# mhozza/covest

Measured on AMD Instinct MI355X. Metric: grid-point log-likelihood evals/s, repeat model, 10k-bin hist, higher is better.
Workload: dtype f64

## Files before the change

covest_amd/csrc/abi_grid.cpp:

```cpp
#include "host.h"

using namespace covest;

namespace covest {

int grid_stage_begin(covest_grid *g, size_t bytes, StageSlot &slot)
{
    if (!g->async_uploads) {
        SharedStage &ss = shared_stage();
        slot.shared_hold = std::unique_lock<std::mutex>(ss.mu);
        HIP_TRY(ss.buf.reserve(bytes));
        slot.ptr = ss.buf.as<char>();
        return COVEST_OK;
    }
    const size_t at = (g->stage_off + 63) / 64 * 64;
    if (at + bytes > g->stage.cap) {
        if (g->stage.ptr)
            g->stage_retired.push_back(std::move(g->stage));
        HIP_TRY(g->stage.reserve(std::max<size_t>(2 * (at + bytes), 1 << 18)));
        slot.ptr = g->stage.as<char>();
        g->stage_off = bytes;
        return COVEST_OK;
    }
    slot.ptr = g->stage.as<char>() + at;
// ... 15 lines not shown

}

namespace {

int check_grid_args(const covest_model *m, int32_t n_axes, const double *const *axes, const int64_t *axis_len, int64_t flat_begin,
                    int64_t *flat_end, const char *who, int64_t *total_out, int64_t *n_values_out)
{
    if (!axes || !axis_len)
        return fail(COVEST_E_INVALID, std::string(who) + ": null argument");
    if (n_axes != m->n_par)
        return fail(COVEST_E_INVALID, std::string(who) + ": n_axes must equal the model's param_count");
    int64_t total = 1, n_values = 0;
    for (int d = 0; d < n_axes; ++d) {
        if (axis_len[d] < 1 || !axes[d])
            return fail(COVEST_E_INVALID, std::string(who) + ": every axis needs at least one value");
        if (total > (int64_t)1 << 40)
            return fail(COVEST_E_INVALID, std::string(who) + ": grid too large");
        total *= axis_len[d];
        n_values += axis_len[d];
    }
    if (*flat_end < 0)
        *flat_end = total;
    if (flat_begin < 0 || flat_begin > *flat_end || *flat_end > total)
        return fail(COVEST_E_INVALID, std::string(who) + ": bad flat index range");
    *total_out = total;
    *n_values_out = n_values;
    return COVEST_OK;
}

struct GridArena {
    size_t ctl, axes, table;
    size_t staged_bytes;
    size_t ll, idx, word, partial_val, partial_idx, result, bytes;
    GridArena(int64_t n_values, int64_t nq, int64_t n)
    {
        const size_t n_pts = (size_t)(n > 0 ? n : 1);
        ctl = 0;
        axes = 8;
        table = axes + (size_t)n_values * sizeof(double);
        staged_bytes = (table + (size_t)nq * sizeof(int32_t) + 7) / 8 * 8;
        ll = staged_bytes;
        idx = ll + n_pts * sizeof(double);
        word = idx + n_pts * sizeof(int64_t);
        partial_val = word + n_pts * sizeof(unsigned long long);
        partial_idx = partial_val + kArgminBlocks * sizeof(double);
        result = partial_idx + kArgminBlocks * sizeof(int64_t);
        bytes = result + sizeof(ArgminResult);
    }
};

int stage_inputs(covest_grid *g, const GridArena &a, int32_t n_axes, const double *const *axes, const int64_t *axis_len,
                 const std::vector<int32_t> &table, int64_t n, char **inputs)
{
    const void *arena_before = g->arena.ptr;
    const bool counter_clean = g->counter_clean;
    HIP_TRY(g->arena.reserve(a.bytes));
    char *base = g->arena.as<char>();
    StageSlot slot;
    const int src = grid_stage_begin(g, a.staged_bytes, slot);
    if (src != COVEST_OK)
        return src;
    char *stage = slot.ptr;
    std::memset(stage, 0, a.staged_bytes);
    double *sa = reinterpret_cast<double *>(stage + a.axes);
    for (int d = 0; d < n_axes; ++d) {
        std::copy(axes[d], axes[d] + axis_len[d], sa);
        sa += axis_len[d];
    }
    if (!table.empty())
        std::memcpy(stage + a.table, table.data(), table.size() * sizeof(int32_t));
    if (g->async_uploads && n <= kArgminSmall) {
        *inputs = stage;
        if (!(counter_clean && g->arena.ptr == arena_before && g->sub_ctl.ptr == base + a.ctl)) {
            HIP_TRY(hipMemsetAsync(base + a.ctl, 0, 8, nullptr));
            g->upload_pending = true;
        }
        return COVEST_OK;
    }
    *inputs = base;
    return grid_stage_commit(g, slot, base, a.staged_bytes);
}

void bind_views(covest_grid *g, const GridArena &a, char *inputs, int32_t n_axes, const int64_t *axis_len, int64_t flat_begin)
{
    char *base = g->arena.as<char>();
    g->axes.ptr = inputs + a.axes;
    g->sub_ctl.ptr = base + a.ctl;
    g->t_table.ptr = inputs + a.table;
    g->ll.ptr = base + a.ll;
    g->sub_index.ptr = base + a.idx;
    g->sub_word.ptr = base + a.word;
    g->partial_val.ptr = base + a.partial_val;
    g->partial_idx.ptr = base + a.partial_idx;
    g->result.ptr = base + a.result;
    PointSource &src = g->src;
    src = PointSource{};
    src.is_grid = 1;
    src.flat_begin = flat_begin;
    int64_t off = 0;
    for (int d = 0; d < kMaxParams; ++d) {
        g->len[d] = src.len[d] = d < n_axes ? axis_len[d] : 1;
        src.axis[d] = d < n_axes ? g->axes.as<double>() + off : nullptr;
        if (d < n_axes)
            off += axis_len[d];
    }
    if (g->model->n_par == 5)
        src.t_table = g->t_table.as<int32_t>();
}

struct TMinus1Sums {
    double block, q;
};

TMinus1Sums sum_t_minus_1(const std::vector<int32_t> &table, int64_t nq, int64_t flat_begin, int64_t flat_end)
{
    std::vector<double> prefix((size_t)nq + 1, 0.0);
    for (int64_t i = 0; i < nq; ++i)
        prefix[(size_t)i + 1] = prefix[(size_t)i] + (double)(table[(size_t)i] > 1 ? table[(size_t)i] - 1 : 0);
    auto upto = [&](int64_t flat) {
        return (double)(flat / nq) * prefix[(size_t)nq] + prefix[(size_t)(flat % nq)];
    };
    return {upto(flat_end) - upto(flat_begin), prefix[(size_t)nq]};
}

// ... 64 lines not shown
        pinned_block_give(g->result_host);
        g->result_host = nullptr;
    }
    g->arena.release();
    g->plan_buf.release();
    g->axis_buf.release();
    g->axis_host.release();
    for (covest_grid::Part &part : g->long_parts)
        part.buf.release();
    g->long_parts.clear();
    g->long_q_orig.release();
    g->long_partial.release();
    for (hipEvent_t e : g->ev_begin)
        (void)hipEventDestroy(e);
    for (hipEvent_t e : g->ev_end)
        (void)hipEventDestroy(e);
    g->ev_begin.clear();
    g->ev_end.clear();
}

extern "C" {

int covest_grid_create(covest_model *m, int32_t n_axes, const double *const *axes,
                       const int64_t *axis_len, int64_t flat_begin, int64_t flat_end,
                       covest_grid **out)
{
    if (!m || !out)
        return fail(COVEST_E_INVALID, "covest_grid_create: null argument");
    *out = nullptr;
    covest_grid *g = new (std::nothrow) covest_grid();
    if (!g)
        return fail(COVEST_E_NOMEM, "covest_grid_create: out of host memory");
    g->model = m;
    std::lock_guard<std::mutex> guard(m->lock);
    DeviceGuard dev_guard(m->device);
    int rc = dev_guard.status();
    if (rc == COVEST_OK)
        rc = grid_configure(g, n_axes, axes, axis_len, flat_begin, flat_end, "covest_grid_create");
    if (rc != COVEST_OK) {
        grid_release(g);
        delete g;
        return rc;
    }
    *out = g;
    return COVEST_OK;
}

int covest_grid_reset(covest_grid *g, int32_t n_axes, const double *const *axes, const int64_t *axis_len,
                      int64_t flat_begin, int64_t flat_end)
{
    if (!g)
        return fail(COVEST_E_INVALID, "covest_grid_reset: null grid");
    covest_model *m = g->model;
    std::lock_guard<std::mutex> guard(m->lock);
    DeviceGuard dev_guard(m->device);
    if (dev_guard.status() != COVEST_OK)
        return dev_guard.status();
    if (g->last_stream || g->evaluated)
        HIP_TRY(hipStreamSynchronize(g->last_stream));
    if (g->upload_pending && !g->evaluated)
        HIP_TRY(hipStreamSynchronize(nullptr));
    g->upload_pending = false;
    g->stage_retired.clear();
    g->async_uploads = true;
    return grid_configure(g, n_axes, axes, axis_len, flat_begin, flat_end, "covest_grid_reset");
}
// ... 75 lines not shown
    for (unsigned long long w : words) {
        const long long unit = sub_units16(w) ? 16 : 1;
        const long long len = ((long long)sub_last(w) - (long long)sub_first(w) + 1) * unit;
        sum += (double)len;
        mx = std::max(mx, len);
        mn = std::min(mn, len);
        first_sum += (long long)sub_first(w) * unit;
    }
    std::fprintf(stderr, "covest_grid_eval: rows named per point: min %lld mean %.1f max %lld; mean first row %.1f\n", mn,
                 sum / queued, mx, (double)first_sum / queued);
    if (!g->src.t_table)
        return COVEST_OK;
    const int64_t n_q = g->src.len[2] * g->src.len[3] * g->src.len[4];
    std::vector<int32_t> tt((size_t)n_q);
    std::vector<int64_t> idx(queued);
    HIP_TRY(hipMemcpy(tt.data(), g->src.t_table, (size_t)n_q * sizeof(int32_t), hipMemcpyDeviceToHost));
    HIP_TRY(hipMemcpy(idx.data(), g->sub_index.ptr, (size_t)queued * sizeof(int64_t), hipMemcpyDeviceToHost));
    long long tmin = 1 << 30, tmax = 0;
    double tsum = 0;
    long long hist[6] = {0, 0, 0, 0, 0, 0};
    for (int64_t i : idx) {
        const long long T = tt[(size_t)((g->src.flat_begin + i) % n_q)];
        tmin = std::min(tmin, T);
        tmax = std::max(tmax, T);
        tsum += (double)T;
        hist[T <= 16 ? 0 : T <= 32 ? 1 : T <= 64 ? 2 : T <= 128 ? 3 : T <= 256 ? 4 : 5]++;
    }
    std::fprintf(stderr, "covest_grid_eval: threshold_o of the queued points: min %lld mean %.1f max %lld; <=16 %lld <=32 %lld <=64 %lld <=128 %lld <=256 %lld more %lld\n",
                 tmin, tsum / queued, tmax, hist[0], hist[1], hist[2], hist[3], hist[4], hist[5]);
    return COVEST_OK;
}
#endif

static int grid_eval(covest_grid *g, int32_t kernel, void *stream, bool scan, double scan_start)
{
    if (!g)
        return fail(COVEST_E_INVALID, "covest_grid_eval: null grid");
    if (!g->configured)
        return fail(COVEST_E_INVALID, "covest_grid_eval: the last covest_grid_reset of this handle failed; reset it again");
    covest_model *m = g->model;
    const int kern = resolve_kernel(m, kernel, g);
    if (kern < 0)
        return kern;
    std::lock_guard<std::mutex> guard(m->lock);
    DeviceGuard dev_guard(m->device);
    int rc = dev_guard.status();
    if (rc != COVEST_OK)
        return rc;
    LaunchRecordScope record(g->record);
    hipStream_t st = static_cast<hipStream_t>(stream);
    const int64_t n = g->flat_end - g->flat_begin;
    if (g->upload_pending && st != nullptr && g->upload_ev)
        HIP_TRY(hipStreamWaitEvent(st, g->upload_ev, 0));
    hipEvent_t bracket_end = nullptr;
    rc = bracket_begin(g, st, &bracket_end);
    if (rc != COVEST_OK)
        return rc;
    HIP_TRY(launch_ll(m, kern, g->src, n, g->ll.as<double>(), sub_list_of(m, g->has_plan ? g->t_max : 2, g->sub_index.ptr, g->sub_word.ptr, g->sub_ctl.ptr), st,
                      &g->last_kernel, g));
    g->last_kernel_id = kern;
    if (bracket_end)
        HIP_TRY(hipEventRecord(bracket_end, st));
#ifdef COVEST_DIAG
    rc = report_queue(g, st, n);
    if (rc != COVEST_OK)
        return rc;
#endif
    if (!g->result_host) {
        static_assert(sizeof(ArgminResult) <= 64 && 64 + sizeof(ScanRecords) <= kPinnedBlockBytes, "pinned block");
        g->result_host = static_cast<ArgminResult *>(pinned_block_take());
        if (!g->result_host)
            return fail(COVEST_E_NOMEM, "covest_grid_eval: no page-locked memory for the result");
    }
    g->scan_valid = scan && n >= 1 && n <= kArgminSmall;
    if (g->scan_valid)
        HIP_TRY(launch_argmin_scan(g->ll.as<double>(), n, g->flat_begin, scan_start, g->result.as<ArgminResult>(), g->result_host,
                                   g->scan_host(), g->sub_ctl.as<unsigned>(), st));
    else
        HIP_TRY(launch_argmin(g->ll.as<double>(), n, g->flat_begin, g->partial_val.as<double>(),
                              g->partial_idx.as<int64_t>(), g->result.as<ArgminResult>(), g->result_host, g->sub_ctl.as<unsigned>(), st));
    g->last_stream = st;
    g->evaluated = true;
    return COVEST_OK;
}

int covest_grid_eval(covest_grid *g, int32_t kernel, void *stream) { return grid_eval(g, kernel, stream, false, 0.0); }

int covest_grid_eval_scan(covest_grid *g, int32_t kernel, void *stream, double start_min)
{
    return grid_eval(g, kernel, stream, true, start_min);
}

int covest_grid_scan(covest_grid *g, int32_t cap, int64_t *index, double *negll, int32_t *n_records, int32_t *truncated)
{
    if (!g || !n_records || !truncated || cap < 0 || (cap > 0 && (!index || !negll)))
        return fail(COVEST_E_INVALID, "covest_grid_scan: bad argument");
    if (!g->evaluated)
        return fail(COVEST_E_INVALID, "covest_grid_scan: covest_grid_eval_scan has not run");
    DeviceGuard dev_guard(g->model->device);
    int rc = dev_guard.status();
    if (rc != COVEST_OK)
        return rc;
    HIP_TRY(hipStreamSynchronize(g->last_stream));
    *n_records = 0;
    *truncated = 1;
    if (!g->scan_valid)
        return COVEST_OK;
    const ScanRecords *sr = g->scan_host();
    const int32_t have = sr->n;
    *truncated = (sr->truncated || have > cap) ? 1 : 0;
// ... 145 lines not shown
```

covest_amd/csrc/argmin.hip:

```cpp
#include <hip/hip_runtime.h>

#include <algorithm>

#include "cand.h"
#include "direct_point.h"
#include "fastmath.h"
#include "kernels.h"
#include "wave.h"

namespace covest {

namespace {

__device__ __forceinline__ Cand block_best(Cand c)
{
    __shared__ double sv[16];
    __shared__ int64_t si[16];
    c = wave_best(c);
    const int lane = threadIdx.x & (kWave - 1), w = threadIdx.x / kWave;
    if (lane == 0) {
        sv[w] = c.v;
        si[w] = c.i;
    }
    __syncthreads();
// ... 130 lines not shown
                                if (u >= n)
                                    break;
                                if (idx[u] >= cur_end) {
                                    if (cur_end > 0)
                                        pj += wave_bcast(b_o, cur_end - S) * inner;
                                    inner = 0.0;
                                    while (idx[u] >= cur_end)
                                        cur_end += S;
                                }
                                inner += t[u];
                            }
                        }
                        if (cur_end > 0)
                            pj += wave_bcast(b_o, cur_end - S) * inner;
                    }
                }
            }
            if (NW > 1) {
                pj_part[wave][lane] = pj;
                __syncthreads();
                pj = ((pj_part[0][lane] + pj_part[1][lane]) + pj_part[2][lane]) + pj_part[3][lane];
            }
            const bool fix = counted && pj < list.p_clamp;
            const double contrib = fix ? h * ((pj <= 0.0 ? -INFINITY : log(pj)) - list.log_p_clamp) : 0.0;
            uint64_t todo = __ballot(fix);
            while (todo) {
                const int kk = __builtin_ctzll(todo);
                todo &= todo - 1;
                value += wave_bcast(contrib, kk);
            }
            if (NW > 1)
                __syncthreads();
        }
        if (lane == 0 && wave == 0)
            ll[pt] = value;
    }
}

template <int SC>
__global__ __launch_bounds__(256) void ll_fix_basic_packed_kernel(const DevModel m, const int32_t n_tiles, const int32_t n_items,
                                                                  const double *__restrict__ tile_dbl,
                                                                  const int32_t *__restrict__ tile_int, const PointSource src,
                                                                  double *__restrict__ ll, const SubList list)
{
    const unsigned count = __builtin_amdgcn_readfirstlane(*list.count);
    if (count == 0)
        return;
    __shared__ __attribute__((aligned(16))) double log_tab[kLogTableDoubles];
    load_log_table(log_tab);
    const TileView tv = tile_view_from(n_tiles, n_items, tile_dbl, tile_int);
    const int lane = threadIdx.x & (kWave - 1);
    constexpr int S = SC;
    constexpr int G = kWave / S;
    const int g = lane / S, s = lane - g * S;
    const bool in_group = g < G;
    const int first_lane = (in_group ? g : 0) * S;
    const double comb_s = m.comb[s];
    const int64_t n_rows_table = (int64_t)tv.n_tiles * kTileBins;
    const unsigned wave_global = blockIdx.x * (blockDim.x / kWave) + threadIdx.x / kWave;
    const unsigned n_waves = gridDim.x * (blockDim.x / kWave);
    bool have = false;
    int64_t pt = 0, row_first = 0, row_last = -1;
    double par[kMaxParams] = {0, 0, 0, 0, 0};
    int T = 0;
    double value = 0.0, h_n = 0.0, key_n = 0.0, nlg_n = 0.0;
    auto fetch_row = [&](int64_t r0, double &h, double &key, double &nlg) {
        const int64_t row = row_first + r0 + s;
        const int bin = (have && row <= row_last && row < n_rows_table) ? tv.row_bin[row] : -1;
// ... 37 lines not shown
            nd = -log_trunc_norm(x, lx, log_tab);
        }
        if (!live)
            a_s = 0.0;
        const int64_t my_rows = have ? row_last - row_first + 1 : 0;
        int64_t most = my_rows;
#pragma unroll
        for (int off = 32; off >= 1; off >>= 1)
            most = max(most, __shfl_xor(most, off, kWave));
        for (int64_t r0 = 0; r0 < most; r0 += S) {
            const double h = h_n, key = key_n, nlg = nlg_n;
            if (r0 + S < most)
                fetch_row(r0 + S, h_n, key_n, nlg_n);
            const bool counted = h != 0.0;
            double pj = 0.0;
#pragma unroll
            for (int t = 0; t < S; ++t) {
                const double a_t = __shfl(a_s, first_lane + t, kWave);
                const double lx_t = __shfl(lx, first_lane + t, kWave);
                const double nd_t = __shfl(nd, first_lane + t, kWave);
                const double term = a_t * exp(fma(key, lx_t, nd_t + nlg));
                pj += (a_t != 0.0) ? term : 0.0;
            }
            const bool fix = counted && pj < list.p_clamp;
            const double contrib = fix ? h * ((pj <= 0.0 ? -INFINITY : log(pj)) - list.log_p_clamp) : 0.0;
#pragma unroll
            for (int t = 0; t < S; ++t) {
                const double c_t = __shfl(contrib, first_lane + t, kWave);
                const bool f_t = __shfl((int)fix, first_lane + t, kWave) != 0;
                if (f_t)
                    value += c_t;
            }
        }
        if (have && s == 0)
            ll[pt] = value;
    }
}

__device__ __forceinline__ void publish(Cand c, int64_t flat_begin, ArgminResult *__restrict__ result,
                                        ArgminResult *__restrict__ host_mirror)
{
    ArgminResult r;
    r.min_negll = c.v;
    r.index = (c.i == INT64_MAX) ? -1 : c.i;
    r.pair[0] = c.v;
    r.pair[1] = (c.i == INT64_MAX) ? -1.0 : (double)(flat_begin + c.i);
    *result = r;
    if (host_mirror)
        *host_mirror = r;
}

__global__ __launch_bounds__(256) void argmin_stage2(const double *__restrict__ pv,
                                                     const int64_t *__restrict__ pi, int n_part, int64_t flat_begin,
                                                     ArgminResult *__restrict__ result, ArgminResult *__restrict__ host_mirror,
                                                     unsigned *__restrict__ queue_count)
{
    if (threadIdx.x == 0 && queue_count)
        *queue_count = 0;
    Cand c;
    c.v = INFINITY;
    c.i = INT64_MAX;
    for (int i = threadIdx.x; i < n_part; i += blockDim.x) {
        Cand o;
        o.v = pv[i];
        o.i = pi[i];
        c = better(c, o);
    }
    c = block_best(c);
// ... 10 lines not shown
        double v[4];
#pragma unroll
        for (int u = 0; u < 4; ++u) {
            const int64_t i = base + (int64_t)u * kSmallThreads;
            v[u] = i < n ? -ll[i] : INFINITY;
        }
#pragma unroll
        for (int u = 0; u < 4; ++u) {
            const int64_t i = base + (int64_t)u * kSmallThreads;
            if (i < n)
                take(i, v[u]);
        }
    }
}

__global__ __launch_bounds__(kSmallThreads) void argmin_small(const double *__restrict__ ll, int64_t n, int64_t flat_begin,
                                                             ArgminResult *__restrict__ result, ArgminResult *__restrict__ host_mirror,
                                                             unsigned *__restrict__ queue_count)
{
    if (threadIdx.x == 0 && queue_count)
        *queue_count = 0;
    Cand c;
    c.v = INFINITY;
    c.i = INT64_MAX;
    small_grid_values(ll, n, [&](int64_t i, double v) {
        if (v < c.v) {
            c.v = v;
            c.i = i;
        }
    });
    c = block_best(c);
    if (threadIdx.x == 0)
        publish(c, flat_begin, result, host_mirror);
}

__global__ __launch_bounds__(kSmallThreads) void argmin_scan_small(const double *__restrict__ ll, int64_t n, int64_t flat_begin,
                                                                  double start, ArgminResult *__restrict__ result,
                                                                  ArgminResult *__restrict__ host_mirror,
                                                                  ScanRecords *__restrict__ scan, unsigned *__restrict__ queue_count)
{
    constexpr int NW = kSmallThreads / kWave;
    extern __shared__ double vals[];
    __shared__ double wave_min[NW];
    __shared__ int wave_cnt[NW];
    const int tid = threadIdx.x, lane = tid & (kWave - 1), w = tid / kWave;
    if (tid == 0 && queue_count)
        *queue_count = 0;
    Cand c;
    c.v = INFINITY;
    c.i = INT64_MAX;
    small_grid_values(ll, n, [&](int64_t i, double v) {
        vals[i] = v;
        if (v < c.v) {
            c.v = v;
            c.i = i;
        }
    });
    c = block_best(c);
    if (tid == 0)
        publish(c, flat_begin, result, host_mirror);
    const int chunk = (int)((n + kSmallThreads - 1) / kSmallThreads);
    const int lo = min((int)n, tid * chunk), hi = min((int)n, lo + chunk);
    double m = INFINITY;
    for (int i = lo; i < hi; ++i)
        m = vals[i] < m ? vals[i] : m;
    double incl = m;
// ... 29 lines not shown
            pre += o;
    }
    if (lane == kWave - 1)
        wave_cnt[w] = pre;
    __syncthreads();
    int at = pre - cnt, total = 0;
    for (int k = 0; k < NW; ++k) {
        if (k < w)
            at += wave_cnt[k];
        total += wave_cnt[k];
    }
    run = run0;
    for (int i = lo; i < hi; ++i)
        if (vals[i] < run) {
            run = vals[i];
            if (at < kScanCap) {
                scan->rec[at].index = flat_begin + i;
                scan->rec[at].negll = run;
            }
            ++at;
        }
    if (tid == 0) {
        scan->start = start;
        scan->truncated = total > kScanCap ? 1 : 0;
        scan->n = min(total, kScanCap);
    }
}

}

const char *const kFixVariantNames[kFixVariants] = {"fix_basic_packed<8>",  "fix_basic_packed<16>", "fix_basic_packed<24>",
                                                    "fix_basic_packed<32>", "fix_list<2,1>",        "fix_list<5,1>"};
const char *const kArgminVariantNames[kArgminVariants] = {"argmin_small", "argmin_stage1+2", "argmin_scan_small"};

hipError_t launch_argmin_scan(const double *ll, int64_t n, int64_t flat_begin, double start, ArgminResult *result,
                              ArgminResult *host_mirror, ScanRecords *scan, unsigned *queue_count, hipStream_t stream)
{
    if (n > kArgminSmall || n < 1)
        return hipErrorInvalidValue;
    const size_t lds = (size_t)n * sizeof(double);
    static bool raised[64] = {false};
    int dev = 0;
    if (hipGetDevice(&dev) != hipSuccess || dev < 0 || dev >= 64)
        dev = 0;
    if (!raised[dev]) {
        hipError_t e = hipFuncSetAttribute(reinterpret_cast<const void *>(&argmin_scan_small),
                                           hipFuncAttributeMaxDynamicSharedMemorySize, (int)(kArgminSmall * sizeof(double)));
        if (e != hipSuccess)
            return e;
        raised[dev] = true;
    }
    record_launch(kArgminVariantNames[2]);
    hipLaunchKernelGGL(argmin_scan_small, dim3(1), dim3(kSmallThreads), lds, stream, ll, n, flat_begin, start, result, host_mirror, scan,
                       queue_count);
    return hipGetLastError();
}

hipError_t launch_ll_fix_list(const DevModel &m, const TileView &tv, const PointSource &src, double *ll,
                              const SubList &list, hipStream_t stream, int64_t n_points)
{
    const dim3 grid((unsigned)std::min<int64_t>(2048, std::max<int64_t>(64, n_points > 0 ? (n_points + 3) / 4 : 2048))), block(256);
    const int packed_blocks = (int)std::min<int64_t>(512, std::max<int64_t>(16, n_points > 0 ? (n_points + 31) / 32 : 512));
    if (m.kind == 0 && m.n_err <= 32 && m.n_err % 8 == 0) {
        auto go = [&](auto kern) {
            hipLaunchKernelGGL(kern, dim3(packed_blocks), block, 0, stream, m, tv.n_tiles, tv.n_items, tv.dbl_base, tv.int_base, src,
                               ll, list);
        };
        record_launch(kFixVariantNames[m.n_err == 8 ? 0 : m.n_err == 16 ? 1 : m.n_err == 24 ? 2 : 3]);
        switch (m.n_err) {
        case 8: go(ll_fix_basic_packed_kernel<8>); break;
        case 16: go(ll_fix_basic_packed_kernel<16>); break;
        case 24: go(ll_fix_basic_packed_kernel<24>); break;
        default: go(ll_fix_basic_packed_kernel<32>); break;
        }
    } else if (m.kind == 0) {
        record_launch(kFixVariantNames[4]);
        hipLaunchKernelGGL((ll_fix_list_kernel<2, 1>), grid, block, 0, stream, m, tv.n_tiles, tv.n_items, tv.dbl_base,
                           tv.int_base, src, ll, list);
    } else {
        record_launch(kFixVariantNames[5]);
        hipLaunchKernelGGL((ll_fix_list_kernel<5, 1>), grid, block, 0, stream, m, tv.n_tiles, tv.n_items, tv.dbl_base,
                           tv.int_base, src, ll, list);
    }
    return hipGetLastError();
}

hipError_t launch_argmin(const double *ll, int64_t n, int64_t flat_begin, double *partial_val, int64_t *partial_idx,
                         ArgminResult *result, ArgminResult *host_mirror, unsigned *queue_count, hipStream_t stream)
{
    if (n <= kArgminSmall) {
        record_launch(kArgminVariantNames[0]);
        hipLaunchKernelGGL(argmin_small, dim3(1), dim3(kSmallThreads), 0, stream, ll, n, flat_begin, result, host_mirror, queue_count);
        return hipGetLastError();
    }
    const int blocks = (int)std::min<int64_t>(kArgminBlocks, std::max<int64_t>(1, (n + 255) / 256));
    record_launch(kArgminVariantNames[1]);
    hipLaunchKernelGGL(argmin_stage1, dim3(blocks), dim3(256), 0, stream, ll, n, partial_val, partial_idx);
    hipLaunchKernelGGL(argmin_stage2, dim3(1), dim3(256), 0, stream, partial_val, partial_idx, blocks, flat_begin, result,
                       host_mirror, queue_count);
    return hipGetLastError();
}

}
```

covest_amd/csrc/direct_point.h:

```cpp
#pragma once
#include <hip/hip_runtime.h>

#include "device_model.h"
#include "point_fetch.h"
#include "tiles.h"
#include "wave.h"

namespace covest {


constexpr unsigned long long kSubFieldMask = 0xFFFFFull;
constexpr double kClampPerTerm = 7e-317;
constexpr double kZeroSteps = 0.12;
constexpr double kGridStep = 4.94065645841246544e-324;
constexpr double zero_steps_scaled(double two_to_sh) { return kZeroSteps * (kGridStep * two_to_sh); }

__host__ __device__ inline unsigned long long sub_word(unsigned first, unsigned last, bool units16)
{
    return (1ull << 62) | ((unsigned long long)(units16 ? 1 : 0) << 60) | ((unsigned long long)last << 20) |
           (unsigned long long)first;
}
struct SubList {
    double p_clamp;
    double log_p_clamp;
    unsigned *count;
    int64_t *index;
    unsigned long long *word;
    int64_t index_offset;
#ifdef COVEST_DIAG
    int diag_class;
#endif
#ifdef __HIPCC__
    __device__ __forceinline__ void push(int64_t idx, unsigned long long w) const
    {
        const unsigned at = atomicAdd(count, 1u);
        index[at] = idx;
        word[at] = w;
    }
#endif
};

__host__ __device__ inline unsigned sub_first(unsigned long long w) { return (unsigned)(w & kSubFieldMask); }
__host__ __device__ inline unsigned sub_last(unsigned long long w) { return (unsigned)((w >> 20) & kSubFieldMask); }
__host__ __device__ inline bool sub_units16(unsigned long long w) { return ((w >> 60) & 1) != 0; }

constexpr int kDirectBinsPerLane = 4;

template <int P>
__device__ __forceinline__ double strict_pj_wave(const DevModel &m, const double *par, int T, double key, double neg_lgam)
{
    const int lane = threadIdx.x & (kWave - 1);
    const int S = m.n_err;
    const int OT = kWave / S;
    const int s = lane % S;
    const int og = lane / S;
    const bool lane_in_tile = og < OT;
    const double lam = error_class_rate(m, par[0], par[1], s);
    const double comb_s = m.comb[s];
    double p = 0.0;
    for (int o0 = 1; o0 < T; o0 += OT) {
        const int o = o0 + og;
// ... 157 lines not shown
```

covest_amd/csrc/host.h:

```cpp
#pragma once
#include <hip/hip_runtime.h>

#include <algorithm>
#include <cmath>
#include <cstdio>
#include <cstdlib>
#include <cstring>
#include <deque>
#include <limits>
#include <mutex>
#include <new>
#include <string>
#include <vector>

#include "../../include/covest_amd.h"
#include "device_model.h"
#include "direct_point.h"
#include "kernels.h"

namespace covest {

int set_error(int code, const std::string &msg);
inline int fail(int code, const std::string &msg) { return set_error(code, msg); }
int fail_hip(hipError_t e, const char *what);
// ... 161 lines not shown
    int hist_max = 0;
    int64_t key_max = 0;
    double rows_contracted = 0.0, keys_logged = 0.0;
    double low_tile_share = 0.0;
    bool tail_is_zero = true;
    double threshold = 0.0;
    bool has_threshold = true;
    DevBuf bins_eval, bins_all;
    DevBuf tiles_buf;
    TileView tv{};
    bool has_tiles = false;
    DevBuf ws_params, ws_t, ws_out, ws_p;
    DevBuf ws_plan, ws_plan2, ws_partial, ws_items;
    HostBuf ws_stage, ws_result;
    DevBuf ws_sub_index, ws_sub_word, ws_sub_ctl;
    LaunchRecord record;
    std::mutex lock;
};

struct covest_grid {
    covest_model *model = nullptr;
    int64_t len[kMaxParams] = {1, 1, 1, 1, 1};
    int64_t flat_begin = 0, flat_end = 0;
    PointSource src{};
    DevBuf arena, plan_buf;
    DevBuf axis_buf;
    HostBuf axis_host;
    struct View {
        void *ptr = nullptr;
        template <class T> T *as() const { return static_cast<T *>(ptr); }
        void release() { ptr = nullptr; }
    };
    View axes, t_table, ll, sub_index, sub_word, sub_ctl, partial_val, partial_idx, result;
    FactoredPlan plan{};
    bool has_plan = false;
    bool has_short_part = false;
    struct Part {
        DevBuf buf;
        FactoredPlan plan{};
    };
    std::vector<Part> long_parts;
    int32_t n_long_tiles = 0;
    int32_t n_shared_tiles = 0;
    std::vector<int32_t> long_q_orig_host;
    DevBuf long_q_orig, long_partial;
    int t_max = 2;
    double q_sum_t_minus_1 = 0.0;
    double contract_flops_per_row = 0.0;
    double sum_t_minus_1 = 0.0;
    LaunchRecord record;
    const char *last_kernel = "none";
    int last_kernel_id = 0;
    hipStream_t last_stream = nullptr;
    ArgminResult *result_host = nullptr;
    ScanRecords *scan_host() const { return reinterpret_cast<ScanRecords *>(reinterpret_cast<char *>(result_host) + 64); }
    bool scan_valid = false;
    bool counter_clean = false;
    HostBuf stage;
    std::vector<HostBuf> stage_retired;
    size_t stage_off = 0;
    bool async_uploads = false;
    bool upload_pending = false;
    hipEvent_t upload_ev = nullptr;
    bool evaluated = false;
    bool configured = false;
    bool profiling = false;
// ... 78 lines not shown
```

covest_amd/csrc/kernels.h:

```cpp
#pragma once
#include <hip/hip_runtime_api.h>

#include "device_model.h"
#include "direct_point.h"
#include "tiles.h"

namespace covest {

struct LaunchRecord {
    struct Entry {
        const char *name;
        int64_t launches;
    };
    struct Plan {
        int32_t n_threads, n_buf, ld, n_qblocks, shared_tiles, n_pass, list_mode;
        bool long_part;
    };
    Entry entries[16];
    int n_entries = 0;
    Plan plans[8];
    int n_plans = 0;
    void clear() { n_entries = n_plans = 0; }
};
void record_launch(const char *name, int64_t launches = 1);
// ... 9 lines not shown
extern const char *const kBasicVariantNames[kBasicVariants];
extern const char *const kFixVariantNames[kFixVariants];
extern const char *const kArgminVariantNames[kArgminVariants];

hipError_t launch_ll_direct(const DevModel &m, const PointSource &src, int64_t n, double *out_ll,
                            double *out_p, hipStream_t stream, bool ref_overflow = false);

hipError_t launch_ll_basic(const DevModel &m, const TileView &tv, const PointSource &src, int64_t n,
                           double *out_ll, const SubList &sub_list, hipStream_t stream);

hipError_t launch_ll_factored(const DevModel &m, const TileView &tv, const FactoredPlan &plan,
                              double *out_ll, const SubList &sub_list, hipStream_t stream);

hipError_t launch_ll_finish_partials(const DevModel &m, const TileView &tv, const double *partial,
                                     const int32_t *first_item, const double *point_par, const int32_t *point_T,
                                     int64_t n_points, double *out_ll, hipStream_t stream);

hipError_t launch_ll_finish_dense(const DevModel &m, const TileView &tv, const PointSource &src, const double *partial,
                                  int64_t ce_first, int64_t n_ce, int64_t n_cols, const int32_t *q_orig, int64_t n_q,
                                  int64_t flat_end, double *out_ll, hipStream_t stream);

hipError_t launch_ll_fix_list(const DevModel &m, const TileView &tv, const PointSource &src, double *ll,
                              const SubList &list, hipStream_t stream, int64_t n_points = 0);

constexpr int kArgminBlocks = 1024;
struct ArgminResult {
    double min_negll;
    int64_t index;
    double pair[2];
};
constexpr int64_t kArgminSmall = 16384;
hipError_t launch_argmin(const double *ll, int64_t n, int64_t flat_begin, double *partial_val, int64_t *partial_idx,
                         ArgminResult *result, ArgminResult *host_mirror, unsigned *queue_count, hipStream_t stream);

constexpr int kScanCap = 120;
struct ScanRecords {
    int32_t n;
    int32_t truncated;
    double start;
    struct {
        int64_t index;
        double negll;
    } rec[kScanCap];
};
hipError_t launch_argmin_scan(const double *ll, int64_t n, int64_t flat_begin, double start, ArgminResult *result,
                              ArgminResult *host_mirror, ScanRecords *scan, unsigned *queue_count, hipStream_t stream);

struct AxisMinPlan {
    int32_t n_kept, n_red;
    int32_t last_kept, first_kept;
    int64_t klen[3], kstride[3];
    int64_t rlen[3], rstride[3];
    int64_t n_cells, n_red_total;
    int64_t flat_begin, flat_end;
    int64_t lead_lo, lead_hi;
    int64_t r_begin, r_end;
    int64_t n_slices, per_slice;
};
bool axis_min_plan(const int64_t *len, int n_axes, uint32_t keep_mask, int64_t flat_begin, int64_t flat_end, AxisMinPlan *out);
hipError_t launch_axis_min(const AxisMinPlan &p, const double *ll, double *partial_val, int64_t *partial_idx, double *out_val,
                           int64_t *out_idx, hipStream_t stream);

constexpr int kDerivOpg = 3;
int ll_deriv_segments(const DevModel &m);
size_t ll_deriv_partial_bytes(const DevModel &m, int order, int64_t n);
hipError_t launch_ll_deriv(const DevModel &m, int order, const PointSource &src, int64_t n, double *partial, double *out_ll,
// ... 83 lines not shown
```

covest_amd/csrc/ll_basic.hip:

```cpp
#include <hip/hip_runtime.h>

#include <type_traits>

#include "direct_point.h"
#include "fastmath.h"
#include "kernels.h"
#include "point_fetch.h"
#include "streams.h"
#include "wave.h"

namespace covest {

namespace {

template <int S, bool TAIL, int BD>
__device__ __forceinline__ void ll_basic_body(const DevModel &m, const int32_t n_tiles, const int32_t n_items,
                                              const double *__restrict__ tile_dbl, const int32_t *__restrict__ tile_int,
                                              const PointSource &src, const int64_t n, double *__restrict__ out_ll,
                                              const SubList &sub_list)
{
    const TileView tv = tile_view_from(n_tiles, n_items, tile_dbl, tile_int);
    __shared__ __attribute__((aligned(16))) double log_tab[kLogTableDoubles];
    const int64_t pt = (int64_t)blockIdx.x * blockDim.x + threadIdx.x;
    const bool live = pt < n;
    const int64_t ptc = live ? pt : n - 1;

    double par[kMaxParams];
    int T;
    fetch_point<2>(src, ptc, par, T);
    load_log_table(log_tab);
    __syncthreads();
    clamp_point<2>(m, par);
    const bool finite = isfinite(par[0]) && isfinite(par[1]);

    double lam[S];
    error_class_rates<S>(m, par[0], par[1], lam);
    {
        const double jl = tv.last_key[0], x0 = lam[0];
        bool sure = false;
        if (jl > 0.0)
            sure = finite && par[1] < 0.75 && x0 >= 1.0 && x0 <= jl - 1.0 &&
                   fma(jl, fast_log(x0, log_tab), -(x0 + tv.last_key[1])) < -765.5;
        bool leave = !__any(finite && !sure);
#ifdef COVEST_DIAG
        leave = leave && sub_list.diag_class == 0;
#endif
        if (leave) {
            if (live)
                out_ll[pt] = finite ? -INFINITY : NAN;
            return;
        }
    }
    extern __shared__ double anchors[];
    StreamSet<S, LdsAnchors<S>> st;
    st.an.mine = anchors + threadIdx.x;
    st.an.stride = BD;
    st.init(m, lam, 1, finite, log_tab, log_tab);

    double acc_ll = 0.0;
    uint64_t dead = 0;
    unsigned long long subw = 0;
    const double p_clamp = sub_list.p_clamp;
    CompSum acc_sp = {0.0, 0.0};

    const double clamp_s = p_clamp * kBasicScale;
    const double zero_s = zero_steps_scaled(kBasicScale);
    double tile_sp = 0.0;
    auto account = [&](double ps, double h, int row) {
        if (TAIL)
            tile_sp += ps;
        if (h != 0.0) {
            const double xs[1] = {max_raw(ps, clamp_s)};
            double lg[1];
            fast_log_bits_n<1, 5, kBasicShift>(xs, lg, log_tab);
            acc_ll = fma(h, lg[0], acc_ll);
            const uint64_t low = __ballot(ps < clamp_s) & ~dead;
            if (__builtin_expect(low != 0, 0)) {
                const bool zero = ps <= zero_s;
                dead |= __ballot(zero);
                if (!zero && ps < clamp_s)
                    subw = subw ? sub_word(sub_first(subw), (unsigned)row, false) : sub_word((unsigned)row, (unsigned)row, false);
            }
// ... 172 lines not shown
            }
            do_tile(std::integral_constant<int, 1>{}, t, skipped, ll_done);
            skipped = false;
        }
    }

    double tail_term = 0.0;
    if (TAIL) {
        double sp = (acc_sp.hi + acc_sp.lo) * (1.0 / kBasicScale);
        if (!(sp < 1.0))
            sp = 1.0;
        if (sp < 1.0)
            tail_term = m.tail * log(1.0 - sp);
    }
    if ((dead >> (threadIdx.x & (kWave - 1))) & 1)
        acc_ll = isnan(acc_ll) ? acc_ll : -INFINITY;
    double ll = acc_ll + tail_term;
    if (!finite) {
        ll = NAN;
        subw = 0;
    }
    if (!isfinite(ll))
        subw = 0;
#ifdef COVEST_DIAG
    if (sub_list.diag_class != 0) {
        ll = sub_list.diag_class == 1 ? diag_class : diag_lp;
        subw = 0;
    }
#endif
    if (live) {
        out_ll[pt] = ll;
        if (subw != 0)
            sub_list.push(pt + sub_list.index_offset, subw);
    }
}

#ifndef COVEST_BASIC_BD
#define COVEST_BASIC_BD 128
#endif
template <bool TAIL>
__global__ __launch_bounds__(COVEST_BASIC_BD) __attribute__((amdgpu_waves_per_eu(TAIL ? 3 : 4, TAIL ? 3 : 4))) void ll_basic_kernel(
    const DevModel m, const int32_t n_tiles, const int32_t n_items, const double *__restrict__ tile_dbl,
    const int32_t *__restrict__ tile_int, const PointSource src, const int64_t n, double *__restrict__ out_ll,
    SubList sub_list)
{
    ll_basic_body<8, TAIL, COVEST_BASIC_BD>(m, n_tiles, n_items, tile_dbl, tile_int, src, n, out_ll, sub_list);
}

template <int S, bool TAIL>
__global__ __launch_bounds__(64) void ll_basic_wide_kernel(const DevModel m, const int32_t n_tiles, const int32_t n_items,
                                                           const double *__restrict__ tile_dbl,
                                                           const int32_t *__restrict__ tile_int, const PointSource src,
                                                           const int64_t n, double *__restrict__ out_ll, SubList sub_list)
{
    ll_basic_body<S, TAIL, 64>(m, n_tiles, n_items, tile_dbl, tile_int, src, n, out_ll, sub_list);
}

}

template <int S, bool TAIL>
void launch_ll_basic_variant(dim3 grid, hipStream_t stream, const DevModel &m, const TileView &tv, const PointSource &part,
                             int64_t cnt, double *out, const SubList &sl)
{
    if (S == 8) {
        const size_t lds8 = (size_t)2 * 8 * COVEST_BASIC_BD * sizeof(double);
        hipLaunchKernelGGL((ll_basic_kernel<TAIL>), grid, dim3(COVEST_BASIC_BD), lds8, stream, m, tv.n_tiles, tv.n_items, tv.dbl_base,
// ... 72 lines not shown
```

covest_amd/csrc/ll_factored.hip:

```cpp
#include <hip/hip_runtime.h>

#include <algorithm>
#include <mutex>
#include <type_traits>

#include "direct_point.h"
#include "fastmath.h"
#include "kernels.h"
#include "point_fetch.h"
#include "streams.h"
#include "wave.h"

namespace covest {

namespace {

typedef double d4 __attribute__((ext_vector_type(4)));

constexpr double kShareScale = 0x1p128;


template <int N, int MU>
__device__ __forceinline__ void contract_step(int i, const double *cur, const int (&a_off)[MU], const int (&cut)[MU],
                                              const double (&r4)[MU], double (&wrun)[MU], d4 (&acc)[MU])
{
    double a[N];
#pragma unroll
    for (int k = 0; k < N; ++k)
        a[k] = cur[a_off[k] + 4 * i];
#pragma unroll
    for (int k = 0; k < N; ++k) {
        const double w = (i < cut[k]) ? wrun[k] : 0.0;
        wrun[k] *= r4[k];
        acc[k] = __builtin_amdgcn_mfma_f64_16x16x4f64(a[k], w, acc[k], 0, 0, 0);
    }
}

[[maybe_unused]] constexpr int kLdWide = 290;
// ... 738 lines not shown
    double *part_lo = Gs + lay_end.part_lo(t_end);
#pragma unroll
    for (int k = 0; k < MU; ++k) {
        double ll = llacc[k];
        const uint64_t nm = __ballot(wfirst[k] != wfirst[k] || wrun[k] != wrun[k]);
        const uint64_t nan_cols_k = ((nm | (nm >> 16) | (nm >> 32) | (nm >> 48)) & 0xFFFFull) * 0x0001000100010001ull;
        if ((nan_cols_k >> lane) & 1)
            ll = NAN;
        if ((dead[k] >> lane) & 1)
            ll = isnan(ll) ? ll : -INFINITY;
        ll += __shfl_xor(ll, 16, kWave);
        ll += __shfl_xor(ll, 32, kWave);
        CompSum sp = spacc[(TAIL && !SPO) ? k : 0];
        if (TAIL && !SPO) {
#pragma unroll
            for (int off = 16; off <= 32; off <<= 1) {
                const double ohi = __shfl_xor(sp.hi, off, kWave);
                const double olo = __shfl_xor(sp.lo, off, kWave);
                double e;
                two_sum(sp.hi, ohi, sp.hi, e);
                sp.lo += olo + e;
            }
        }
        if (lane < 16) {
            const int at = (wave * MU + k) * 16 + lane;
            part_ll[at] = ll;
            if (TAIL && !SPO) {
                part_hi[at] = sp.hi;
                part_lo[at] = sp.lo;
            }
        }
    }
    __syncthreads();
    auto finish_entry = [&](int e, int qt, int e_half, int e_cont, int pslot, int qo_early) __attribute__((always_inline)) {
        const int c = e & 15;
        if (qt < 0 || e_half != 0 || e_cont)
            return;
        const int pe = pslot >= 0 ? pslot * 16 + c : -1;
        const double ll = (part_ll[e] + (pe >= 0 ? part_ll[pe] : 0.0)) + lconst;
        unsigned u_first = sub_rec[2 * e], u_end = sub_rec[2 * e + 1];
        if (pe >= 0) {
            u_first = min(u_first, sub_rec[2 * pe]);
            u_end = max(u_end, sub_rec[2 * pe + 1]);
        }
        const unsigned long long word = u_end ? sub_word(u_first, u_end - 1, true) : 0ull;
        double tail_term = 0.0;
        double hi = 0.0, lo = 0.0;
        if (TAIL) {
            hi = part_hi[e];
            lo = part_lo[e];
            if (pe >= 0 && !SPO) {
                double err;
                two_sum(hi, part_hi[pe], hi, err);
                lo += part_lo[pe] + err;
            }
        }
        const int32_t qo = kEntriesEarly ? qo_early : plan.q_orig[qt * 16 + c];
        if (list_mode == 1) {
            if (qo >= 0) {
                double *o = plan.partial + ((int64_t)ce * n_seg + seg) * 4;
                o[0] = finite ? ll : NAN;
                o[1] = hi;
                o[2] = lo;
                o[3] = __longlong_as_double((long long)(finite ? word : 0ull));
            }
            return;
        }
        if (TAIL) {
            double s = hi + lo;
            if (!(s < 1.0))
                s = 1.0;
            if (s < 1.0)
                tail_term = m.tail * log(1.0 - s);
        }
        if (qo >= 0) {
            const int64_t flat = ce * plan.n_q + qo;
            if (flat >= plan.flat_begin && flat < plan.flat_end) {
                const double v = finite ? ll + tail_term : NAN;
                out_ll[flat - plan.flat_begin] = v;
                if (word != 0 && isfinite(v))
                    sub_list.push(flat - plan.flat_begin, word);
            }
        }
    };
    if (kEntriesEarly) {
#pragma unroll
        for (int u = 0; u < kEntries; ++u)
            if (tid + u * NT < NE)
                finish_entry(tid + u * NT, en_qt[u], en_half[u], en_cont[u], en_pair[u], en_qo[u]);
    } else {
        for (int e = tid; e < NE; e += NT) {
            const int at = wave_block(e / (MU * 16)) * MU + (e / 16) % MU;
            const int qt = plan.unit_tile[at], e_half = plan.unit_half[at], e_cont = plan.unit_cont[at];
            finish_entry(e, qt, e_half, e_cont, plan.unit_pair[at], 0);
        }
    }
#ifdef COVEST_DIAG
    if (plan.diag && (plan.skip_phases & 0x40000) && lane == 0) {
        long long *d = plan.diag + ((int64_t)(blockIdx.x * gridDim.y + blockIdx.y) * NW + wave) * 8;
        const long long end = (long long)clock64();
        d[0] = dgx_1 - dgx_0;
        d[1] = dgx_2 - dgx_1;
        d[2] = dgx_3 - dgx_2;
        d[3] = dgx_4 - dgx_3;
        d[4] = end - dgx_4;
        d[5] = end - dgx_0;
        d[6] = dgx_0;
        d[7] = end;
    }
#endif
}

#ifndef COVEST_FACTORED_VARIANT
template <class ReadPj>
__device__ __forceinline__ double finish_point(const DevModel &m, const TileView &tv, const double *par, int T,
                                               ReadPj read_pj)
{
    const int lane = threadIdx.x & (kWave - 1);
    const int64_t n_rows = (int64_t)tv.n_items * kTileBins;
    double ll = 0.0;
    bool dead = false, poisoned = false;
    CompSum sp = {0.0, 0.0};
    for (int64_t base = 0; base < n_rows; base += kWave) {
        const int64_t row = base + lane;
        const bool valid = row < n_rows;
        const double pj_scaled = valid ? read_pj(row) : 0.0;
        double pj = pj_scaled * (1.0 / kShareScale);
// ... 264 lines not shown
```

Before: 396.8 million.

## Fuse argmin partial reduction into log-likelihood kernels with single-block final pass

The LL kernels now compute per-wave or per-block argmin candidates as they write values. Points that still need the fix-up pass record their corrected negated values in a new fixed-value array. A single-block final kernel then reduces these partials plus the queued fixed values, replacing the separate full argmin pass over the ll array. This avoids re-reading all ll values in return for extra reductions and shared-memory syncs inside the main kernels, plus a larger arena.

```diff
diff --git a/covest_amd/csrc/abi_grid.cpp b/covest_amd/csrc/abi_grid.cpp
--- a/covest_amd/csrc/abi_grid.cpp
+++ b/covest_amd/csrc/abi_grid.cpp
@@ -71,10 +71,11 @@
 struct GridArena {
     size_t ctl, axes, table;
     size_t staged_bytes;
-    size_t ll, idx, word, partial_val, partial_idx, result, bytes;
+    size_t ll, idx, word, fixed, partial_val, partial_idx, result, bytes;
     GridArena(int64_t n_values, int64_t nq, int64_t n)
     {
         const size_t n_pts = (size_t)(n > 0 ? n : 1);
+        const size_t n_part = (size_t)SubList::partials_room((int64_t)n_pts);
         ctl = 0;
         axes = 8;
         table = axes + (size_t)n_values * sizeof(double);
@@ -82,9 +83,10 @@
         ll = staged_bytes;
         idx = ll + n_pts * sizeof(double);
         word = idx + n_pts * sizeof(int64_t);
-        partial_val = word + n_pts * sizeof(unsigned long long);
-        partial_idx = partial_val + kArgminBlocks * sizeof(double);
-        result = partial_idx + kArgminBlocks * sizeof(int64_t);
+        fixed = word + n_pts * sizeof(unsigned long long);
+        partial_val = fixed + n_pts * sizeof(double);
+        partial_idx = partial_val + n_part * sizeof(double);
+        result = partial_idx + n_part * sizeof(int64_t);
         bytes = result + sizeof(ArgminResult);
     }
 };
@@ -130,6 +132,7 @@
     g->ll.ptr = base + a.ll;
     g->sub_index.ptr = base + a.idx;
     g->sub_word.ptr = base + a.word;
+    g->sub_fixed.ptr = base + a.fixed;
     g->partial_val.ptr = base + a.partial_val;
     g->partial_idx.ptr = base + a.partial_idx;
     g->result.ptr = base + a.result;
@@ -260,6 +263,10 @@
     if (!g)
         return fail(COVEST_E_NOMEM, "covest_grid_create: out of host memory");
     g->model = m;
+    {
+        const char *v = std::getenv("COVEST_KERNEL_ARGMIN_FROM_VALUES");
+        g->argmin_from_values = v && *v && std::strcmp(v, "0") != 0;
+    }
     std::lock_guard<std::mutex> guard(m->lock);
     DeviceGuard dev_guard(m->device);
     int rc = dev_guard.status();
@@ -401,6 +408,21 @@
 }
 #endif
 
+static int64_t argmin_partials_of(const covest_grid *g, int kern, bool scan)
+{
+    if (g->argmin_from_values || scan)
+        return 0;
+    int64_t n_part = 0;
+    if (kern == COVEST_KERNEL_FACTORED) {
+        const FactoredPlan &pl = g->plan;
+        if (g->has_short_part && g->n_long_tiles == 0 && pl.list_mode == 0 && pl.n_qblocks == 1)
+            n_part = pl.ce_end - pl.ce_begin;
+    } else if (kern == COVEST_KERNEL_RECUR && g->model->dm.n_err <= 8) {
+        n_part = (g->flat_end - g->flat_begin + kWave - 1) / kWave;
+    }
+    return n_part >= 1 && n_part <= kArgminPartialsMax ? n_part : 0;
+}
+
 static int grid_eval(covest_grid *g, int32_t kernel, void *stream, bool scan, double scan_start)
 {
     if (!g)
@@ -425,8 +447,15 @@
     rc = bracket_begin(g, st, &bracket_end);
     if (rc != COVEST_OK)
         return rc;
-    HIP_TRY(launch_ll(m, kern, g->src, n, g->ll.as<double>(), sub_list_of(m, g->has_plan ? g->t_max : 2, g->sub_index.ptr, g->sub_word.ptr, g->sub_ctl.ptr), st,
-                      &g->last_kernel, g));
+    SubList sub = sub_list_of(m, g->has_plan ? g->t_max : 2, g->sub_index.ptr, g->sub_word.ptr, g->sub_ctl.ptr);
+    const int64_t n_part = argmin_partials_of(g, kern, scan);
+    if (n_part) {
+        sub.partials_for = n > 0 ? n : 1;
+        if (sub.fixed_val() != g->sub_fixed.as<double>() || sub.part_val() != g->partial_val.as<double>() ||
+            sub.part_idx() != g->partial_idx.as<int64_t>())
+            return fail(COVEST_E_INVALID, "covest_grid_eval: the arena's layout and SubList's differ");
+    }
+    HIP_TRY(launch_ll(m, kern, g->src, n, g->ll.as<double>(), sub, st, &g->last_kernel, g));
     g->last_kernel_id = kern;
     if (bracket_end)
         HIP_TRY(hipEventRecord(bracket_end, st));
@@ -445,6 +474,8 @@
     if (g->scan_valid)
         HIP_TRY(launch_argmin_scan(g->ll.as<double>(), n, g->flat_begin, scan_start, g->result.as<ArgminResult>(), g->result_host,
                                    g->scan_host(), g->sub_ctl.as<unsigned>(), st));
+    else if (n_part)
+        HIP_TRY(launch_argmin_partials(sub, n_part, g->flat_begin, g->result.as<ArgminResult>(), g->result_host, st));
     else
         HIP_TRY(launch_argmin(g->ll.as<double>(), n, g->flat_begin, g->partial_val.as<double>(),
                               g->partial_idx.as<int64_t>(), g->result.as<ArgminResult>(), g->result_host, g->sub_ctl.as<unsigned>(), st));
diff --git a/covest_amd/csrc/argmin.hip b/covest_amd/csrc/argmin.hip
--- a/covest_amd/csrc/argmin.hip
+++ b/covest_amd/csrc/argmin.hip
@@ -186,8 +186,11 @@
             if (NW > 1)
                 __syncthreads();
         }
-        if (lane == 0 && wave == 0)
+        if (lane == 0 && wave == 0) {
             ll[pt] = value;
+            if (list.partials_for)
+                list.fixed_val()[at] = -value;
+        }
     }
 }
 
@@ -291,8 +294,11 @@
                     value += c_t;
             }
         }
-        if (have && s == 0)
+        if (have && s == 0) {
             ll[pt] = value;
+            if (list.partials_for)
+                list.fixed_val()[base + (unsigned)g] = -value;
+        }
     }
 }
 
@@ -369,6 +375,44 @@
     c = block_best(c);
     if (threadIdx.x == 0)
         publish(c, flat_begin, result, host_mirror);
+}
+
+__device__ __forceinline__ Cand scan_pairs(const double *__restrict__ v, const int64_t *__restrict__ idx, int64_t n, Cand c)
+{
+    for (int64_t base = threadIdx.x; base < n; base += 4 * kSmallThreads) {
+        Cand o[4];
+#pragma unroll
+        for (int u = 0; u < 4; ++u) {
+            const int64_t i = base + (int64_t)u * kSmallThreads;
+            o[u].v = i < n ? v[i] : INFINITY;
+            o[u].i = i < n ? idx[i] : INT64_MAX;
+        }
+#pragma unroll
+        for (int u = 0; u < 4; ++u)
+            if (o[u].v < INFINITY)
+                c = better(c, o[u]);
+    }
+    return c;
+}
+
+__global__ __launch_bounds__(kSmallThreads) void argmin_partials_final(const double *__restrict__ pv, const int64_t *__restrict__ pi,
+                                                                      int64_t n_part, const double *__restrict__ fixed_val,
+                                                                      const int64_t *__restrict__ fixed_idx,
+                                                                      unsigned *__restrict__ queue_count, int64_t flat_begin,
+                                                                      ArgminResult *__restrict__ result,
+                                                                      ArgminResult *__restrict__ host_mirror)
+{
+    const unsigned count = *queue_count;
+    Cand c;
+    c.v = INFINITY;
+    c.i = INT64_MAX;
+    c = scan_pairs(pv, pi, n_part, c);
+    c = scan_pairs(fixed_val, fixed_idx, (int64_t)count, c);
+    c = block_best(c);
+    if (threadIdx.x == 0) {
+        *queue_count = 0;
+        publish(c, flat_begin, result, host_mirror);
+    }
 }
 
 __global__ __launch_bounds__(kSmallThreads) void argmin_scan_small(const double *__restrict__ ll, int64_t n, int64_t flat_begin,
@@ -464,6 +508,7 @@
 const char *const kFixVariantNames[kFixVariants] = {"fix_basic_packed<8>",  "fix_basic_packed<16>", "fix_basic_packed<24>",
                                                     "fix_basic_packed<32>", "fix_list<2,1>",        "fix_list<5,1>"};
 const char *const kArgminVariantNames[kArgminVariants] = {"argmin_small", "argmin_stage1+2", "argmin_scan_small"};
+const char *const kArgminPartialsName = "partials_argmin";
 
 hipError_t launch_argmin_scan(const double *ll, int64_t n, int64_t flat_begin, double start, ArgminResult *result,
                               ArgminResult *host_mirror, ScanRecords *scan, unsigned *queue_count, hipStream_t stream)
@@ -517,6 +562,18 @@
     return hipGetLastError();
 }
 
+hipError_t launch_argmin_partials(const SubList &list, int64_t n_part, int64_t flat_begin, ArgminResult *result,
+                                  ArgminResult *host_mirror, hipStream_t stream)
+{
+    if (n_part < 1 || n_part > SubList::partials_room(list.partials_for) || list.partials_for < 1 || !list.word || !list.index ||
+        !list.count)
+        return hipErrorInvalidValue;
+    record_launch(kArgminPartialsName);
+    hipLaunchKernelGGL(argmin_partials_final, dim3(1), dim3(kSmallThreads), 0, stream, list.part_val(), list.part_idx(), n_part,
+                       list.fixed_val(), list.index, list.count, flat_begin, result, host_mirror);
+    return hipGetLastError();
+}
+
 hipError_t launch_argmin(const double *ll, int64_t n, int64_t flat_begin, double *partial_val, int64_t *partial_idx,
                          ArgminResult *result, ArgminResult *host_mirror, unsigned *queue_count, hipStream_t stream)
 {
diff --git a/covest_amd/csrc/direct_point.h b/covest_amd/csrc/direct_point.h
--- a/covest_amd/csrc/direct_point.h
+++ b/covest_amd/csrc/direct_point.h
@@ -27,6 +27,15 @@
     int64_t *index;
     unsigned long long *word;
     int64_t index_offset;
+    int64_t partials_for;
+    static constexpr int64_t kPartialsMin = 1024, kPartialsMax = 16384;
+    __host__ __device__ static int64_t partials_room(int64_t capacity)
+    {
+        return capacity < kPartialsMin ? kPartialsMin : capacity > kPartialsMax ? kPartialsMax : capacity;
+    }
+    __host__ __device__ double *fixed_val() const { return reinterpret_cast<double *>(word + partials_for); }
+    __host__ __device__ double *part_val() const { return fixed_val() + partials_for; }
+    __host__ __device__ int64_t *part_idx() const { return reinterpret_cast<int64_t *>(part_val() + partials_room(partials_for)); }
 #ifdef COVEST_DIAG
     int diag_class;
 #endif
diff --git a/covest_amd/csrc/host.h b/covest_amd/csrc/host.h
--- a/covest_amd/csrc/host.h
+++ b/covest_amd/csrc/host.h
@@ -217,6 +217,8 @@
         void release() { ptr = nullptr; }
     };
     View axes, t_table, ll, sub_index, sub_word, sub_ctl, partial_val, partial_idx, result;
+    View sub_fixed;
+    bool argmin_from_values = false;
     FactoredPlan plan{};
     bool has_plan = false;
     bool has_short_part = false;
diff --git a/covest_amd/csrc/kernels.h b/covest_amd/csrc/kernels.h
--- a/covest_amd/csrc/kernels.h
+++ b/covest_amd/csrc/kernels.h
@@ -65,6 +65,12 @@
 constexpr int64_t kArgminSmall = 16384;
 hipError_t launch_argmin(const double *ll, int64_t n, int64_t flat_begin, double *partial_val, int64_t *partial_idx,
                          ArgminResult *result, ArgminResult *host_mirror, unsigned *queue_count, hipStream_t stream);
+
+constexpr int64_t kArgminPartialsMax = 16384;
+static_assert(SubList::kPartialsMin == kArgminBlocks && SubList::kPartialsMax == kArgminPartialsMax, "direct_point.h lays the partials out");
+extern const char *const kArgminPartialsName;
+hipError_t launch_argmin_partials(const SubList &list, int64_t n_part, int64_t flat_begin, ArgminResult *result,
+                                  ArgminResult *host_mirror, hipStream_t stream);
 
 constexpr int kScanCap = 120;
 struct ScanRecords {
diff --git a/covest_amd/csrc/ll_basic.hip b/covest_amd/csrc/ll_basic.hip
--- a/covest_amd/csrc/ll_basic.hip
+++ b/covest_amd/csrc/ll_basic.hip
@@ -2,6 +2,7 @@
 
 #include <type_traits>
 
+#include "cand.h"
 #include "direct_point.h"
 #include "fastmath.h"
 #include "kernels.h"
@@ -48,6 +49,10 @@
         if (leave) {
             if (live)
                 out_ll[pt] = finite ? -INFINITY : NAN;
+            if (sub_list.partials_for && live && (threadIdx.x & (kWave - 1)) == 0) {
+                sub_list.part_val()[(pt + sub_list.index_offset) / kWave] = INFINITY;
+                sub_list.part_idx()[(pt + sub_list.index_offset) / kWave] = INT64_MAX;
+            }
             return;
         }
     }
@@ -286,6 +291,20 @@
         out_ll[pt] = ll;
         if (subw != 0)
             sub_list.push(pt + sub_list.index_offset, subw);
+    }
+    if (sub_list.partials_for) {
+        Cand c;
+        c.v = INFINITY;
+        c.i = INT64_MAX;
+        if (live && subw == 0 && -ll < INFINITY) {
+            c.v = -ll;
+            c.i = pt + sub_list.index_offset;
+        }
+        c = wave_best(c);
+        if (live && (threadIdx.x & (kWave - 1)) == 0) {
+            sub_list.part_val()[(pt + sub_list.index_offset) / kWave] = c.v;
+            sub_list.part_idx()[(pt + sub_list.index_offset) / kWave] = c.i;
+        }
     }
 }
 
diff --git a/covest_amd/csrc/ll_factored.hip b/covest_amd/csrc/ll_factored.hip
--- a/covest_amd/csrc/ll_factored.hip
+++ b/covest_amd/csrc/ll_factored.hip
@@ -4,6 +4,7 @@
 #include <mutex>
 #include <type_traits>
 
+#include "cand.h"
 #include "direct_point.h"
 #include "fastmath.h"
 #include "kernels.h"
@@ -808,6 +809,9 @@
         }
     }
     __syncthreads();
+    Cand best;
+    best.v = INFINITY;
+    best.i = INT64_MAX;
     auto finish_entry = [&](int e, int qt, int e_half, int e_cont, int pslot, int qo_early) __attribute__((always_inline)) {
         const int c = e & 15;
         if (qt < 0 || e_half != 0 || e_cont)
@@ -854,8 +858,15 @@
             if (flat >= plan.flat_begin && flat < plan.flat_end) {
                 const double v = finite ? ll + tail_term : NAN;
                 out_ll[flat - plan.flat_begin] = v;
-                if (word != 0 && isfinite(v))
+                if (word != 0 && isfinite(v)) {
                     sub_list.push(flat - plan.flat_begin, word);
+                } else if (-v < INFINITY) {
+                    const int64_t at = flat - plan.flat_begin;
+                    if (-v < best.v || (-v == best.v && at < best.i)) {
+                        best.v = -v;
+                        best.i = at;
+                    }
+                }
             }
         }
     };
@@ -869,6 +880,27 @@
             const int at = wave_block(e / (MU * 16)) * MU + (e / 16) % MU;
             const int qt = plan.unit_tile[at], e_half = plan.unit_half[at], e_cont = plan.unit_cont[at];
             finish_entry(e, qt, e_half, e_cont, plan.unit_pair[at], 0);
+        }
+    }
+    if (list_mode == 0 && sub_list.partials_for) {
+        best = wave_best(best);
+        double *cand_v = reinterpret_cast<double *>(&rowc[0][0]);
+        long long *cand_i = reinterpret_cast<long long *>(&rowc[1][0]);
+        static_assert(NW <= 2 * kTileBins, "a candidate a wave");
+        if (lane == 0) {
+            cand_v[wave] = best.v;
+            cand_i[wave] = best.i;
+        }
+        __syncthreads();
+        if (wave == 0) {
+            Cand r;
+            r.v = lane < NW ? cand_v[lane] : INFINITY;
+            r.i = lane < NW ? (int64_t)cand_i[lane] : INT64_MAX;
+            r = wave_best(r);
+            if (lane == 0) {
+                sub_list.part_val()[blockIdx.x] = r.v;
+                sub_list.part_idx()[blockIdx.x] = r.i;
+            }
         }
     }
 #ifdef COVEST_DIAG
```

Measured after the change: 395.7 million. About the same (-0.3%).
